# cuulee/reporter

Measured on AMD Instinct MI355X. Metric: GPS probes matched/sec (whole node), higher is better.
Workload: dtype f64; 1 GPU; c2; graph=metro, nodes=1048576, directed_edges=3527937, osmlr_segments=1361487, traces_per_gpu=10000, streams=1, device_batches=1, output_segments=1688548

## Files before the change

### reporter_amd/csrc/otr_device.h

```cpp
#pragma once
#include <hip/hip_runtime.h>
#include <stdint.h>

#include "../../include/otr_graph_format.h"

#define OTR_KMAX 64
#define OTR_MODES 3
#define OTR_WAVE 64
#define OTR_COUNTERS 24

namespace otr {

constexpr double kMetersPerDeg = 20037581.187 / 180.0;

struct MatchParams {
  double sigma_z;
  double beta;
  double max_route_distance_factor;
  double breakage_distance;
  double interpolation_distance;
  double search_radius;
  double max_search_radius;
  double gps_accuracy;
  double max_route_time_factor;
  double turn_penalty_factor;
  double speed_kph;
  double queue_kph;
  double inv2s2;
  double inv_beta;
  int32_t kmax;
  int32_t pad;
};

struct ModeParams {
  MatchParams m[OTR_MODES];
  double delta;
};

constexpr double kMaxBreakage = 30000.0;
constexpr int64_t kTbMax = 131070;
constexpr uint32_t kTcCap = 2097151;

__host__ __device__ inline int32_t time_bound_ds(const MatchParams& p, int64_t dt) {
  if (!(p.max_route_time_factor > 0.0) || dt <= 0) return -1;
  const double b = floor(p.max_route_time_factor * (double)dt * 10.0);
  return b <= (double)kTbMax ? (int32_t)b : -1;
}

__host__ __device__ inline int turn_from_back(int back, int hb_begin) {
  int td = hb_begin - back;
  td += td < 0 ? 360 : 0;
  return td <= 180 ? td : 360 - td;
}
__host__ __device__ inline int heading_back(int ha_end) { return ha_end >= 180 ? ha_end - 180 : ha_end + 180; }
__host__ __device__ inline int turn_degree(int ha_end, int hb_begin) {
  return turn_from_back(heading_back(ha_end), hb_begin);
}

struct DevGraph {
  const uint32_t* node_row;
  const uint32_t* rev_row;
  const uint32_t* rev_edge;
  const uint32_t* edge_src;
  const uint32_t* edge_dst;
  const float* edge_len;
  const uint32_t* edge_attr;
  const uint32_t* edge_shape;
  const uint32_t* edge_seg;
  const uint32_t* edge_way;
  const int2* shape_ll;
  const unsigned long long* seg_id;
  const uint32_t* seg_len;
  const uint32_t* cell_row;
  const uint32_t* cell_edge;
  const uint4* cell_rec;
  const uint4* edge_pack;
  const uint4* eprep;
  const uint4* adj;
  const uint32_t* node_minin;
  const uint32_t* len_mm;
  const int2* node_ll;
  const uint32_t* adj_t;
  const uint32_t* edge_t;
  uint32_t adj_t_stride, edge_t_stride;
  const short2* edge_head;
  const uint2* adj_e;
  const uint4* erec;
  const uint32_t* erec_t;
  size_t erec_stride;
  uint32_t n_nodes, n_edges, n_segments, grid_rows, grid_cols;
  double grid_min_lat, grid_min_lon, grid_cell_deg;
  __device__ const uint32_t* et(int mode) const { return edge_t + (size_t)mode * edge_t_stride; }
};

__host__ __device__ inline double cos_deg(double deg) {
  double x = deg * (3.14159265358979323846 / 180.0);
  double x2 = x * x;
  double r = -1.0 / 1124000727777607680000.0;
  r = r * x2 + 1.0 / 2432902008176640000.0;
  r = r * x2 - 1.0 / 6402373705728000.0;
  r = r * x2 + 1.0 / 20922789888000.0;
  r = r * x2 - 1.0 / 87178291200.0;
  r = r * x2 + 1.0 / 479001600.0;
  r = r * x2 - 1.0 / 3628800.0;
  r = r * x2 + 1.0 / 40320.0;
  r = r * x2 - 1.0 / 720.0;
  r = r * x2 + 1.0 / 24.0;
  r = r * x2 - 1.0 / 2.0;
  r = r * x2 + 1.0;
  return r;
}

__host__ __device__ inline double gc_dist(double lat1, double lon1, double lat2, double lon2) {
  double x = (lon1 - lon2) * kMetersPerDeg * cos_deg(0.5 * (lat1 + lat2));
  double y = (lat1 - lat2) * kMetersPerDeg;
  return sqrt(x * x + y * y);
}

__host__ __device__ inline double e6(int32_t v) { return (double)v * 1e-6; }

__host__ __device__ inline double route_bound(const MatchParams& p, double g) {
  double gf = g > p.interpolation_distance ? g : p.interpolation_distance;
  double b = p.max_route_distance_factor * gf;
  return b > p.breakage_distance ? p.breakage_distance : b;
}

__device__ inline uint32_t hmix(uint32_t x) {
  x ^= x >> 16;
  x *= 0x7feb352dU;
  x ^= x >> 15;
  x *= 0x846ca68bU;
  x ^= x >> 16;
  return x;
}

__device__ inline int lane_id() { return (int)__lane_id(); }

__device__ inline int64_t xcd_remap(int64_t b, int64_t per) { return (b & 7) * per + (b >> 3); }

struct XcdQueue {
  int64_t lo, hi;
  unsigned long long* ctr;
  __device__ XcdQueue(unsigned long long* q, int64_t n) {
    const int parts = gridDim.x >= 8 ? 8 : 1;
    const int x = parts == 8 ? (int)(blockIdx.x & 7) : 0;
    const int64_t per = (n + parts - 1) / parts;
    lo = (int64_t)x * per;
    hi = lo + per < n ? lo + per : n;
    ctr = q + 16 * x;
  }
  __device__ unsigned long long claim() {
    unsigned long long v = 0;
    if (threadIdx.x == 0) v = atomicAdd(ctr, 1ull);
    return v;
  }
  __device__ int64_t take(unsigned long long v) const {
    const uint32_t l = (uint32_t)__builtin_amdgcn_readfirstlane((int)(uint32_t)v);
    const uint32_t h = (uint32_t)__builtin_amdgcn_readfirstlane((int)(uint32_t)(v >> 32));
    return lo + (int64_t)(((unsigned long long)h << 32) | l);
  }
  __device__ int64_t next() { return take(claim()); }
};

__device__ inline uint4 ld16(const uint4* p) {
  uint4 r = *p;
  asm volatile("" : "+v"(r.x), "+v"(r.y), "+v"(r.z), "+v"(r.w));
  return r;
}

constexpr int kShards = 64;
constexpr int kCShards = 256;
__device__ inline int cshard() { return (int)(blockIdx.x & (kCShards - 1)); }
constexpr uint32_t kAdjDstMask = 0x0FFFFFFFu;
constexpr uint32_t kAdjMore = 0x80000000u;

// ... 6 lines not shown
```

### reporter_amd/csrc/otr_engine.hip

```cpp
#include <hipcub/hipcub.hpp>

#include <cerrno>
#include <cstdio>
#include <cstring>
#include <fcntl.h>
#include <sys/mman.h>
#include <sys/stat.h>
#include <unistd.h>

#include "otr_engine.h"
#include "otr_kernels.h"
#include "otr_edge.h"
#include "otr_edge1.h"
#include "otr_ingest.h"
#include "otr_launch.h"
#include "otr_points.h"
#include "otr_traversals.h"

namespace otr {
static_assert(kTraceWaves == 4, "grid_trace_rows (otr_launch.h) assumes 4 traces per block");

#define HIPCHK(x)                                                                        \
  do {                                                                                   \
    hipError_t e_ = (x);                                                                 \
    if (e_ != hipSuccess) {                                                              \
      if (err) *err = std::string("HIP error: ") + hipGetErrorString(e_) + " at " #x;    \
      return OTR_DEVICE_ERROR;                                                           \
    }                                                                                    \
  } while (0)

void finalize_params(MatchParams* p) {
  p->inv2s2 = 1.0 / (p->sigma_z * p->sigma_z * 2.0);
  p->inv_beta = 1.0 / p->beta;
  if (p->kmax > OTR_KMAX) p->kmax = OTR_KMAX;
  if (p->kmax < 1) p->kmax = 1;
}

const char* check_params(const MatchParams& p) {
  if (!(p.breakage_distance >= 0.0 && p.breakage_distance <= kMaxBreakage))
    return "breakage_distance must be within [0, 30000] m";
  if (!(p.max_route_distance_factor >= 0.0) || !(p.max_route_distance_factor < 1e6))
    return "max_route_distance_factor must be >= 0";
  if (!(p.max_route_time_factor >= 0.0) || !(p.max_route_time_factor < 1e6)) return "max_route_time_factor must be >= 0";
  if (!(p.turn_penalty_factor >= 0.0) || !(p.turn_penalty_factor <= 1e6)) return "turn_penalty_factor must be within [0, 1e6]";
  if (!(p.sigma_z > 0.0)) return "sigma_z must be > 0";
  if (!(p.beta > 0.0)) return "beta must be > 0";
  if (!(p.search_radius >= 0.0) || !(p.max_search_radius >= 0.0)) return "search_radius must be >= 0";
  if (!(p.interpolation_distance >= 0.0)) return "interpolation_distance must be >= 0";
  if (!(p.speed_kph >= 0.0) || !(p.queue_kph >= 0.0)) return "speed_kph and queue_kph must be >= 0";
  return nullptr;
}

ModeParams default_mode_params() {
  ModeParams mp{};
  for (int m = 0; m < OTR_MODES; ++m) {
    MatchParams& p = mp.m[m];
    p.sigma_z = 4.07;
    p.beta = 3.0;
    p.max_route_distance_factor = 5.0;
    p.max_route_time_factor = 2.0;
    p.breakage_distance = 2000.0;
    p.interpolation_distance = 10.0;
    p.search_radius = 50.0;
    p.max_search_radius = 100.0;
    p.gps_accuracy = 5.0;
    p.kmax = 32;
    p.queue_kph = 10.0;
  }
  mp.m[0].turn_penalty_factor = 200.0;
  mp.m[1].turn_penalty_factor = 140.0;
  mp.m[1].speed_kph = 18.0;
  mp.m[1].queue_kph = 5.0;
  mp.m[2].turn_penalty_factor = 100.0;
  mp.m[2].speed_kph = 5.1;
  mp.m[2].queue_kph = 2.0;
  for (int m = 0; m < OTR_MODES; ++m) finalize_params(&mp.m[m]);
  mp.delta = 60.0;
  return mp;
}

static uint32_t edge_time_ds(uint32_t attr, uint32_t len_mm, double speed_cap) {
  double kph = (double)OTR_ATTR_SPEED(attr);
  if (!(kph > 0.0)) kph = 30.0;
  if (speed_cap > 0.0 && speed_cap < kph) kph = speed_cap;
  const double v = (double)len_mm * 0.036 / kph;
  return v < 2.0e9 ? (uint32_t)llround(v) : 2000000000u;
}

static int seg_heading(const int32_t* a, const int32_t* b) {
  const double la1 = (double)a[0] * 1e-6, lo1 = (double)a[1] * 1e-6;
  const double la2 = (double)b[0] * 1e-6, lo2 = (double)b[1] * 1e-6;
  const double m = 20037581.187 / 180.0;
  const double x = (lo2 - lo1) * m * cos_deg(0.5 * (la1 + la2));
// ... 34 lines not shown
};
struct Staged {
  std::vector<void*> allocs;
  bool adopted = false;
  ~Staged() {
    if (!adopted)
      for (void* q : allocs) (void)hipFree(q);
  }
};
}

int engine_configure(const Config& cfg, std::string* err) {
  for (int m = 0; m < OTR_MODES; ++m)
    if (const char* bad = check_params(cfg.mp.m[m])) {
      if (err) *err = std::string("config: ") + bad;
      return OTR_BAD_REQUEST;
    }
  int fd = open(cfg.graph_path.c_str(), O_RDONLY);
  if (fd < 0) {
    if (err) *err = "cannot open graph file " + cfg.graph_path + ": " + strerror(errno);
    return OTR_BAD_REQUEST;
  }
  struct stat st;
  fstat(fd, &st);
  Mapped mf;
  mf.n = (size_t)st.st_size;
  mf.p = mf.n >= sizeof(otr_graph_header) ? mmap(nullptr, mf.n, PROT_READ, MAP_PRIVATE, fd, 0) : MAP_FAILED;
  close(fd);
  if (mf.p == MAP_FAILED) {
    if (err) *err = "cannot map graph file " + cfg.graph_path;
    return OTR_BAD_REQUEST;
  }
  const char* base = (const char*)mf.p;
  otr_graph_header h;
  memcpy(&h, base, sizeof(h));
  if (memcmp(h.magic, OTR_GRAPH_MAGIC, 8) != 0 || h.version != OTR_GRAPH_VERSION ||
      h.array_offset[OTR_A_END] > (uint64_t)st.st_size) {
    if (err) *err = "not an OTR graph file: " + cfg.graph_path;
    return OTR_BAD_REQUEST;
  }
  if (h.n_nodes >= (1u << 28)) {
    if (err) *err = "graph has more than 2^28 nodes";
    return OTR_BAD_REQUEST;
  }
  if (h.n_edges >= (1u << 28)) {
    if (err) *err = "graph has more than 2^28 directed edges";
    return OTR_BAD_REQUEST;
  }
  const uint32_t* dst = (const uint32_t*)(base + h.array_offset[OTR_A_EDGE_DST]);
  const float* lenf = (const float*)(base + h.array_offset[OTR_A_EDGE_LEN]);
  const uint32_t* attr = (const uint32_t*)(base + h.array_offset[OTR_A_EDGE_ATTR]);
  const uint32_t* row = (const uint32_t*)(base + h.array_offset[OTR_A_NODE_ROW]);
  const int32_t* nll = (const int32_t*)(base + h.array_offset[OTR_A_NODE_LL]);
  const uint32_t* eshape = (const uint32_t*)(base + h.array_offset[OTR_A_EDGE_SHAPE]);
  const int32_t* sll = (const int32_t*)(base + h.array_offset[OTR_A_SHAPE_LL]);
  std::vector<uint32_t> len(h.n_edges + 1, 0u);
  for (uint32_t e = 0; e < h.n_edges; ++e) {
    const double mm = (double)lenf[e] * 1000.0;
    if (!(mm >= 0.0 && mm < 2.0e9)) {
      if (err) *err = "graph edge length outside [0, 2000 km)";
      return OTR_BAD_REQUEST;
    }
    len[e] = (uint32_t)std::max(1LL, (long long)llround(mm));
  }
  for (uint32_t u = 0; u < h.n_nodes; ++u)
    if (row[u + 1] < row[u] || row[u + 1] > h.n_edges) {
      if (err) *err = "graph CSR rows are not monotone";
      return OTR_BAD_REQUEST;
    }
  for (uint32_t e = 0; e < h.n_edges; ++e)
    if (dst[e] >= h.n_nodes || eshape[e + 1] < eshape[e] + 2 || eshape[e + 1] > h.n_shape) {
      if (err) *err = "graph edge " + std::to_string(e) + " has a bad end node or shape range";
      return OTR_BAD_REQUEST;
    }
  std::vector<uint32_t> minin(h.n_nodes + 1, 0xFFFFFFFFu);
  for (uint32_t e = 0; e < h.n_edges; ++e) minin[dst[e]] = std::min(minin[dst[e]], len[e]);
  std::vector<uint4> pack(h.n_edges + 1);
  for (uint32_t e = 0; e < h.n_edges; ++e) pack[e] = make_uint4(dst[e], len[e], attr[e], minin[dst[e]]);
  std::vector<uint4> eprep(h.n_edges + 1, make_uint4(0u, 0u, 0u, 0u));
  {
    const uint32_t* srcv = (const uint32_t*)(base + h.array_offset[OTR_A_EDGE_SRC]);
    for (uint32_t e = 0; e < h.n_edges; ++e) eprep[e] = make_uint4(len[e], srcv[e], minin[srcv[e]], dst[e]);
  }
  std::vector<uint4> adj(4ull * h.n_nodes + 4, make_uint4(kAdjDstMask, 0u, 0u, 0u));
  for (uint32_t u = 0; u < h.n_nodes; ++u) {
    const uint32_t deg = row[u + 1] - row[u];
    for (uint32_t k = 0; k < deg && k < 4; ++k) {
      const uint32_t e = row[u] + k;
      adj[4ull * u + k] = make_uint4(dst[e] | ((attr[e] & OTR_ATTR_ACCESS_MASK) << 28), len[e], minin[dst[e]], 0u);
    }
    if (deg > 4) adj[4ull * u + 3].x |= kAdjMore;
  }
  std::vector<uint32_t> et[OTR_MODES], at[OTR_MODES];
  for (int m = 0; m < OTR_MODES; ++m) {
    et[m].assign(h.n_edges + 1, 0u);
    for (uint32_t e = 0; e < h.n_edges; ++e) et[m][e] = edge_time_ds(attr[e], len[e], cfg.mp.m[m].speed_kph);
    at[m].assign(4ull * h.n_nodes + 4, 0u);
    for (uint32_t u = 0; u < h.n_nodes; ++u)
      for (uint32_t k = 0; k < 4 && row[u] + k < row[u + 1]; ++k) at[m][4ull * u + k] = et[m][row[u] + k];
  }
  std::vector<short2> head(h.n_edges + 1, make_short2(0, 0));
  for (uint32_t e = 0; e < h.n_edges; ++e) {
    const uint32_t k0 = eshape[e], k1 = eshape[e + 1];
    int hb = -1, he = -1;
    for (uint32_t k = k0; k + 1 < k1 && hb < 0; ++k) hb = seg_heading(sll + 2ull * k, sll + 2ull * k + 2);
    for (uint32_t k = k1 - 1; k > k0 && he < 0; --k) he = seg_heading(sll + 2ull * k - 2, sll + 2ull * k);
    head[e] = make_short2((short)(hb < 0 ? 0 : hb), (short)(he < 0 ? 0 : he));
  }
  std::vector<uint2> adje(4ull * h.n_nodes + 4, make_uint2(0u, 0u));
  for (uint32_t u = 0; u < h.n_nodes; ++u)
    for (uint32_t k = 0; k < 4 && row[u] + k < row[u + 1]; ++k) {
      const uint32_t e = row[u] + k;
      adje[4ull * u + k] = make_uint2(e, (uint32_t)(uint16_t)head[e].x | ((uint32_t)(uint16_t)head[e].y << 16));
    }
  const size_t es = 4ull * h.n_edges + 4;
  std::vector<uint4> erec(es, make_uint4(kAdjDstMask, 0u, 0u, 0u));
  std::vector<uint32_t> erec_t(es * OTR_MODES, 0u);
  for (uint32_t b = 0; b < h.n_edges; ++b) {
    const uint32_t v = dst[b], deg = row[v + 1] - row[v];
    for (uint32_t k = 0; k < 4; ++k) {
      const uint32_t hend = (uint32_t)(uint16_t)head[b].y << 8;
      if (k >= deg) {
        erec[4ull * b + k] = make_uint4(kAdjDstMask, 0u, hend, v);
        continue;
      }
      const uint32_t e = row[v] + k;
      const uint32_t x = e | ((attr[e] & OTR_ATTR_ACCESS_MASK) << 28) | ((k == 3 && deg > 4) ? kAdjMore : 0u);
      erec[4ull * b + k] =
          make_uint4(x, len[e], (uint32_t)turn_degree((int)head[b].y, (int)head[e].x) | hend, v);
      for (int m = 0; m < OTR_MODES; ++m) erec_t[es * m + 4ull * b + k] = std::min(et[m][e], 0x1FFFFu);
    }
  }
  const uint32_t* cedge = (const uint32_t*)(base + h.array_offset[OTR_A_CELL_EDGE]);
  std::vector<uint4> crec(3 * ((size_t)h.n_cell_entries + 1), make_uint4(0u, 0u, 0u, 0u));
  for (uint64_t q = 0; q < h.n_cell_entries; ++q) {
    const uint32_t e = cedge[q];
    if (e >= h.n_edges) {
      if (err) *err = "graph cell index names a missing edge";
      return OTR_BAD_REQUEST;
    }
    const uint32_t k0 = eshape[e], k1 = eshape[e + 1];
    crec[3 * q] = make_uint4(e, k0, k1, attr[e]);
    uint32_t pt[8] = {0u, 0u, 0u, 0u, 0u, 0u, 0u, 0u};
    for (uint32_t i = 0; i < 4 && k0 + i < k1; ++i) {
      pt[2 * i] = (uint32_t)sll[2ull * (k0 + i)];
      pt[2 * i + 1] = (uint32_t)sll[2ull * (k0 + i) + 1];
    }
    crec[3 * q + 1] = make_uint4(pt[0], pt[1], pt[2], pt[3]);
    crec[3 * q + 2] = make_uint4(pt[4], pt[5], pt[6], pt[7]);
  }
  HIPCHK(hipSetDevice(cfg.device));
  Staged sg;
  bool alloc_ok = true;
  auto upv = [&](const void* src, size_t bytes) -> void* {
    void* d = nullptr;
    if (hipMalloc(&d, bytes ? bytes : 16) != hipSuccess) {
      alloc_ok = false;
      return nullptr;
    }
    sg.allocs.push_back(d);
    if (bytes && hipMemcpy(d, src, bytes, hipMemcpyHostToDevice) != hipSuccess) alloc_ok = false;
    return d;
  };
  auto up = [&](int a, size_t bytes) -> void* { return upv(base + h.array_offset[a], bytes); };
  DevGraph g{};
  g.node_row = (const uint32_t*)up(OTR_A_NODE_ROW, 4ull * (h.n_nodes + 1));
  g.rev_row = (const uint32_t*)up(OTR_A_REV_ROW, 4ull * (h.n_nodes + 1));
  g.node_ll = (const int2*)up(OTR_A_NODE_LL, 8ull * h.n_nodes);
  g.rev_edge = (const uint32_t*)up(OTR_A_REV_EDGE, 4ull * h.n_edges);
  g.edge_src = (const uint32_t*)up(OTR_A_EDGE_SRC, 4ull * h.n_edges);
  g.edge_dst = (const uint32_t*)up(OTR_A_EDGE_DST, 4ull * h.n_edges);
  g.edge_len = (const float*)up(OTR_A_EDGE_LEN, 4ull * h.n_edges);
  g.edge_attr = (const uint32_t*)up(OTR_A_EDGE_ATTR, 4ull * h.n_edges);
  g.edge_shape = (const uint32_t*)up(OTR_A_EDGE_SHAPE, 4ull * (h.n_edges + 1));
  g.edge_seg = (const uint32_t*)up(OTR_A_EDGE_SEG, 4ull * h.n_edges);
  g.edge_way = (const uint32_t*)up(OTR_A_EDGE_WAY, 4ull * h.n_edges);
  g.shape_ll = (const int2*)up(OTR_A_SHAPE_LL, 8ull * h.n_shape);
  g.seg_id = (const unsigned long long*)up(OTR_A_SEG_ID, 8ull * h.n_segments);
  g.seg_len = (const uint32_t*)up(OTR_A_SEG_LEN, 4ull * h.n_segments);
  g.cell_row = (const uint32_t*)up(OTR_A_CELL_ROW, 4ull * (h.n_cells + 1));
  g.cell_edge = (const uint32_t*)up(OTR_A_CELL_EDGE, 4ull * h.n_cell_entries);
  g.len_mm = (const uint32_t*)upv(len.data(), 4ull * len.size());
  g.edge_pack = (const uint4*)upv(pack.data(), sizeof(uint4) * pack.size());
// ... 2681 lines not shown
```

### reporter_amd/csrc/otr_kernels.h

```cpp
#pragma once
#include <cstddef>
#include <type_traits>

#include "otr_device.h"
#include "otr_mincode.h"
#include "otr_pred.h"
#include "otr_report.h"
#include "otr_tilerow.h"

#ifndef OTR_CAP1
#define OTR_CAP1 160
#endif
#ifndef OTR_LOAD1
#define OTR_LOAD1 7
#endif
#ifndef OTR_E1CAP
#define OTR_E1CAP 360
#endif
#ifndef OTR_E1LOAD
#define OTR_E1LOAD 14
#endif

namespace otr {

// ... 693 lines not shown
  const typename LabelT<LM>::T old = atomicMin(&L.lab[sl], nb);
  if (LabelT<LM>::label(nb) < LabelT<LM>::label(old)) {
    knext = nd < knext ? nd : knext;
    if constexpr (OLD) {
      const uint32_t ok = atomicOr(&L.key[sl], kInq);
      if (!(ok & kInq)) return sl;
    } else {
      if (old == LabelT<LM>::kInf) return sl;
    }
  }
  return -1;
}

template <int CAP, bool OLD = false>
__device__ inline int relax_sink(SearchLds<CAP, 0>& L, uint32_t* sink, const Pack& K, uint32_t dw, uint32_t len_mm,
                                 uint32_t time_ds, uint32_t minin, uint32_t pu, uint32_t pd, uint32_t pt,
                                 uint32_t mode_bit, uint32_t& relaxed, uint32_t& knext, bool& isnew, uint32_t& lanew) {
  const bool mode_ok = (((dw >> 28) & 7u) & mode_bit) != 0u;
  relaxed += mode_ok ? 1u : 0u;
  const uint32_t nd = K.d(pu) + len_mm;
  const uint32_t tt = K.t(pu) + time_ds;
  const uint32_t nw = (nd << K.sh) | tt;
  const uint32_t node = dw & kAdjDstMask;
  bool go = mode_ok && nd <= pd && tt <= pt;
  uint32_t* mine = sink + lane_id();
  const uint32_t h0 = hslot<CAP>(node);
  const uint32_t k0 = atomicCAS(go ? &L.key[h0] : mine, kEmpty, node);
  isnew = go && k0 == kEmpty;
  int sl = (go && (k0 == kEmpty || (k0 & kNodeMask) == node)) ? (int)h0 : -1;
  const bool coll = go && sl < 0;
  if (__ballot(coll) != 0ull) {
    if (coll) {
      uint32_t hh = h0;
      for (int probe = 1; probe < CAP; ++probe) {
        hh = hh + 1 == (uint32_t)CAP ? 0u : hh + 1;
        const uint32_t k = atomicCAS(&L.key[hh], kEmpty, node);
        if (k == kEmpty) {
          isnew = true;
          sl = (int)hh;
          break;
        }
        if ((k & kNodeMask) == node) {
          sl = (int)hh;
          break;
        }
      }
      if (sl < 0) {
        L.overflow = 1;
        lanew |= kProbeOut;
      }
    }
  }
  go = go && sl >= 0;
  using MiT = typename SearchLds<CAP, 0>::MiT;
  *((go && isnew) ? &L.mi[sl] : reinterpret_cast<MiT*>(mine)) = SearchLds<CAP, 0>::code(minin);
  const uint32_t old = atomicMin(go ? &L.lab[sl] : mine, nw);
  const bool imp = go && nw < old;
  knext = (imp && nd < knext) ? nd : knext;
  if constexpr (OLD) {
    const uint32_t was = atomicOr(imp ? &L.key[sl] : mine, kInq);
    return (imp && !(was & kInq)) ? sl : -1;
  } else {
    return (imp && old == kNoLabel) ? sl : -1;
  }
}

struct NDump {
  const unsigned long long* in;
  unsigned long long* base;
  unsigned long long* ctr;
  uint32_t words, slots;
#ifdef OTR_FORCE_RETRY
  int stop_rounds;
#endif
};
__host__ __device__ constexpr uint32_t nd_words(int cap) { return 2u + (uint32_t)cap + ((uint32_t)cap + 1u) / 2u; }
#ifndef OTR_ND_IN_MIN
#define OTR_ND_IN_MIN 2048
#endif
#ifndef OTR_ND_OUT_MIN
#define OTR_ND_OUT_MIN 1024
#endif

template <int CAP, int LM, int G = 1, bool RIN = false, bool ROUT = false>
__device__ bool search_run(SearchLds<CAP, LM>* Ls, const DevGraph& g, const Pack& K, uint32_t mode_bit, bool active,
                           uint32_t start, uint32_t pd, uint32_t pt, uint32_t tnode, uint32_t tpart, uint32_t gapT,
                           int n_tgt, unsigned long long* settled, unsigned long long* relaxed,
                           unsigned long long* rounds, unsigned long long* stamps = nullptr, uint32_t* sink = nullptr,
                           const NDump* nd = nullptr, int* dslot = nullptr) {
  using Gr = Grp<G>;
  constexpr bool OLD = old_rounds(G);
  static_assert(!(OLD && (RIN || ROUT)), "the dump and resume code assumes keys without the pending bit");
  constexpr int kMaxKeys = (CAP <= 128 || CAP >= 256) ? (CAP * 7) / 8 : (CAP * OTR_LOAD1) / 8;
  const int gl = Gr::gl();
  using W = typename LabelT<LM>::W;
  SearchLds<CAP, LM>& L = Ls[Gr::g()];
  using Idx = typename SearchLds<CAP, LM>::Idx;
  constexpr int WCAP = SearchLds<CAP, LM>::WCAP;
  const bool timed = K.sh != 0u;
  const uint32_t* adjt = g.adj_t + (size_t)__builtin_ctz(mode_bit) * g.adj_t_stride;
  uint32_t kmin = 0;
  int npend = active ? 1 : 0;
  const bool resume = RIN && LM == 0 && active && nd->in != nullptr;
  const int nres = resume ? (int)nd->in[0] : 0;
  const int nrx = RIN ? Gr::umax(nres) : 0;
  if (RIN && nrx > 0) {
    const unsigned long long* D = nd->in;
    const uint32_t* M = (const uint32_t*)(D + 2 + nres);
    int np = 0;
    for (int base = 0; base < nrx; base += Gr::GL) {
      const int k = base + gl;
      bool pend = false;
      int sl = 0;
      if (k < nres) {
        const unsigned long long e = D[2 + k];
        const uint32_t key = (uint32_t)(e >> 32), node = key & kNodeMask;
        uint32_t h = hslot<CAP>(node);
        for (int probe = 0; probe < CAP; ++probe) {
          if (atomicCAS(&L.key[h], kEmpty, node) == kEmpty) break;
          h = h + 1 == (uint32_t)CAP ? 0u : h + 1;
        }
        sl = (int)h;
        L.key[sl] = key & ~kInq;
        L.lab[sl] = (typename LabelT<LM>::T)(uint32_t)e;
        L.mi[sl] = SearchLds<CAP, LM>::code(M[k]);
        pend = (key & kInq) != 0u;
      }
      const unsigned long long mp = __ballot(pend);
      if (pend && np + Gr::prefix(mp) < SearchLds<CAP, LM>::PCAP) L.pend[np + Gr::prefix(mp)] = (Idx)sl;
      np += Gr::count(mp);
    }
    if (resume && np > SearchLds<CAP, LM>::PCAP) {
      if (gl == 0) L.overflow = 1;
      np = SearchLds<CAP, LM>::PCAP;
    }
    if (resume) {
      npend = np;
      kmin = (uint32_t)D[1];
      if (gl == 0) L.n_keys = nres;
    }
  }
  if (!resume && active && gl == 0) {
    bool isnew;
    const int sl = lds_insert(L, start, &isnew);
    L.mi[sl] = 0;
    L.lab[sl] = LabelT<LM>::make(0u, kEmpty);
    if (OLD) L.key[sl] |= kInq;
    L.pend[0] = (Idx)sl;
  }
  __syncthreads();
  int tslot = -1;
  if (active && gl < n_tgt && tnode != kEmpty) {
    bool isnew;
    tslot = lds_insert(L, tnode, &isnew);
    if (tslot >= 0 && isnew) L.mi[tslot] = SearchLds<CAP, LM>::code(gapT);
  }
  __syncthreads();
  uint32_t my_settled = 0, my_relaxed = 0, my_rounds = 0;
  unsigned long long cyc[4] = {0, 0, 0, 0};
  bool done = !active, grew = false;
#ifdef OTR_FORCE_RETRY
  int force_round = 0;
#endif
  int nkeys = 0;
  constexpr bool AHEAD = !OLD && LM != 1;
  static_assert(!AHEAD || Gr::GL <= SearchLds<CAP, LM>::PCAP, "the first pending chunk lies inside the list");
  const int ts = tslot < 0 ? 0 : tslot;
  int p0 = 0;
  bool ovf = false;
  uint32_t tkey = 0u;
  typename LabelT<LM>::T tlab = LabelT<LM>::kInf;
  if constexpr (AHEAD) {
    nkeys = L.n_keys;
    ovf = L.overflow != 0;
    tkey = L.key[ts];
    tlab = L.lab[ts];
    p0 = (int)L.pend[gl];
  }
  for (;;) {
    OTR_STAMP(t0);
    const int np = done ? 0 : npend;
    OTR_STAMP(t1);
    bool res;
    if constexpr (AHEAD)
      res = done | (gl >= n_tgt) |
            target_test<LM, OLD>(tkey, LabelT<LM>::label(tlab), K, tslot, tpart, gapT, pd, kmin, np == 0);
    else
      res = done | (gl >= n_tgt) | target_resolved<CAP, LM, OLD>(L, K, tslot, tpart, gapT, pd, kmin, np == 0);
    done = done || Gr::mine(__ballot(!res)) == 0ull || np == 0;
    OTR_STAMP(t2);
    cyc[0] += t1 - t0;
    cyc[1] += t2 - t1;
    if (Gr::all(done)) break;
    if (!done && gl == 0) ++my_rounds;
    uint32_t knext = 0xFFFFFFFFu;
    int kept = 0, nw = 0;
    const int npx = OLD ? Gr::umax(np) : 0;
    for (int base = 0; OLD ? base < npx : __ballot(base + gl < np) != 0ull; base += Gr::GL) {
      const int k = base + gl;
      const bool in = k < np;
      int sl;
      if constexpr (AHEAD) {
        int pk = p0;
        if (base != 0) pk = (int)L.pend[k];
        sl = in ? pk : 0;
      } else {
        sl = in ? (int)L.pend[k] : 0;
      }
      const W lb = LabelT<LM>::label(L.lab[sl]);
      const uint32_t key = L.key[sl];
      const uint32_t d = K.d(lb);
      bool take, keep;
      if constexpr (OLD) {
        take = in && (uint64_t)d < (uint64_t)kmin + SearchLds<CAP, LM>::gap(L.mi[sl]);
        take = take && nw + Gr::prefix(__ballot(take)) < WCAP;
        keep = in && !take;
      } else {
        const uint32_t gp = SearchLds<CAP, LM>::gap(L.mi[sl]);
        if constexpr (LM != 2) take = in & in_final32(d, kmin, gp);
        else take = in & ((uint64_t)d < (uint64_t)kmin + gp);
        take = take & (nw + Gr::prefix(__ballot(take)) < WCAP);
        keep = in & !take;
      }
      const unsigned long long mt = __ballot(take), mk = __ballot(keep);
      __syncthreads();
      if (take) {
        L.work[nw + Gr::prefix(mt)] = WorkE<W>{key & kNodeMask, lb};
        L.key[sl] = (key & kNodeMask) | kRel;
      }
      if (keep) L.pend[kept + Gr::prefix(mk)] = (Idx)sl;
      knext = (keep && d < knext) ? d : knext;
      nw += Gr::count(mt);
      kept += Gr::count(mk);
      __syncthreads();
    }
    npend = kept;
    OTR_STAMP(t3);
    cyc[2] += t3 - t2;
    uint32_t tail = 0u;
    uint32_t unread = 0u;
    uint32_t& lanew = AHEAD ? tail : unread;
    const int nwx = OLD ? Gr::umax(4 * nw) : 0;
    for (int base = 0; OLD ? base < nwx : __ballot(base + gl < 4 * nw) != 0ull; base += Gr::GL) {
      const int k = base + gl;
      int psl = -1;
      bool isnew = false;
      if (k < 4 * nw) {
        const WorkE<W> wk = L.work[k >> 2];
        const uint32_t wnode = wk.node;
        const int slot = k & 3;
        if (slot == 0) ++my_settled;
        const uint32_t tq = adjt[4 * (size_t)wnode + slot];
        const uint4 r = ld16(g.adj + 4 * (size_t)wnode + slot);
        const uint32_t tt = timed ? tq : 0u;
        if constexpr (LM == 0) {
#ifdef OTR_NO_SINK
          psl = relax_one<CAP, LM, false, OLD>(L, K, r.x & ~kAdjMore, r.y, tt, r.z, wk.lab, 0u, pd, pt, mode_bit,
                                               my_relaxed, knext, isnew, lanew);
#else
          psl = relax_sink<CAP, OLD>(L, sink, K, r.x & ~kAdjMore, r.y, tt, r.z, wk.lab, pd, pt, mode_bit, my_relaxed,
                                     knext, isnew, lanew);
#endif
        } else {
          const uint32_t e0 = LM == 1 ? g.node_row[wnode] : 0u;
          psl = relax_one<CAP, LM, false, OLD>(L, K, r.x & ~kAdjMore, r.y, tt, r.z, wk.lab, e0 + slot, pd, pt,
                                               mode_bit, my_relaxed, knext, isnew, lanew);
        }
        tail |= slot == 3 ? (r.x & kAdjMore) : 0u;
      }
      nkeys += Gr::count(__ballot(isnew));
      const unsigned long long mp = __ballot(psl >= 0);
#ifndef OTR_NO_SINK
      if constexpr (LM == 0 && G == 1) {
        const int p = npend + Gr::prefix(mp);
        constexpr int PC = SearchLds<CAP, LM>::PCAP;
        *(psl >= 0 ? &L.pend[p < PC ? p : PC - 1] : reinterpret_cast<Idx*>(sink + lane_id())) = (Idx)psl;
      } else
#endif
      if (psl >= 0) {
        const int p = npend + Gr::prefix(mp);
        L.pend[p < SearchLds<CAP, LM>::PCAP ? p : SearchLds<CAP, LM>::PCAP - 1] = (Idx)psl;
      }
      npend += Gr::count(mp);
    }
    if (SearchLds<CAP, LM>::PCAP < CAP && npend > SearchLds<CAP, LM>::PCAP) {
      if (gl == 0) L.overflow = 1;
      npend = SearchLds<CAP, LM>::PCAP;
      ovf = true;
    }
    if (__ballot(AHEAD ? (tail & kAdjMore) != 0u : tail != 0u) != 0ull) {
      if (gl == 0) L.n_pend = npend;
      if (AHEAD && gl == 0) L.n_keys = nkeys;
      __syncthreads();
      for (int base = 0; OLD ? base < nwx : __ballot(base + gl < 4 * nw) != 0ull; base += Gr::GL) {
        const int k = base + gl;
        if (k < 4 * nw && (k & 3) == 3) {
          const WorkE<W> wk = L.work[k >> 2];
          const uint32_t wnode = wk.node;
          if (g.adj[4 * (size_t)wnode + 3].x & kAdjMore)
            for (uint32_t e = g.node_row[wnode] + 4; e < g.node_row[wnode + 1]; ++e) {
              const uint4 pk = ld16(g.edge_pack + e);
              const uint32_t tt = timed ? g.et(__builtin_ctz(mode_bit))[e] : 0u;
              bool isnew;
              const int psl = relax_one<CAP, LM, true, OLD>(L, K, pk.x | ((pk.z & 7u) << 28), pk.y, tt, pk.w, wk.lab, e,
                                                            pd, pt, mode_bit, my_relaxed, knext, isnew, lanew);
              if (psl >= 0) {
                const int p = atomicAdd(&L.n_pend, 1);
                if (p < SearchLds<CAP, LM>::PCAP) L.pend[p] = (Idx)psl;
                else L.overflow = 1;
              }
            }
        }
      }
      __syncthreads();
      npend = L.n_pend;
      if (npend > SearchLds<CAP, LM>::PCAP) npend = SearchLds<CAP, LM>::PCAP;
      if constexpr (AHEAD) {
        nkeys = L.n_keys;
        ovf = ovf || L.overflow != 0;
      }
    }
    __syncthreads();
    if constexpr (AHEAD) {
      tkey = L.key[ts];
      tlab = L.lab[ts];
      p0 = (int)L.pend[gl];
      ovf = ovf || Gr::mine(__ballot((tail & kProbeOut) != 0u)) != 0ull;
    }
    OTR_STAMP(t4);
    cyc[3] += t4 - t3;
    const uint32_t km = Gr::min_u32(knext);
    if (!done) kmin = km;
    const int keys = AHEAD ? nkeys : L.n_keys + nkeys;
    const bool over = AHEAD ? ovf : L.overflow != 0;
    if (!done && (over || keys > kMaxKeys)) {
      grew = !over && keys > kMaxKeys;
      done = true;
    }
#ifdef OTR_FORCE_RETRY
    ++force_round;
    if (ROUT && !done && nd->base != nullptr && nd->stop_rounds > 0 && force_round >= nd->stop_rounds &&
        !over) {
      grew = true;
      done = true;
    }
#endif
    if constexpr (!AHEAD) __syncthreads();
    if (done && active && gl == 0 && (keys > kMaxKeys || grew)) L.overflow = 1;
  }
  if constexpr (AHEAD) {
    if (gl == 0) L.n_keys = nkeys;
  } else {
    if (gl == 0) L.n_keys += nkeys;
  }
  if (ROUT) *dslot = -1;
  if (ROUT && LM == 0 && __ballot(grew && active && nd->base != nullptr) != 0ull) {
    int v = 0;
    if (grew && active && nd->base != nullptr && gl == 0) v = (int)atomicAdd(nd->ctr, 1ull);
    v = __shfl(v, 0, Gr::GL);
    const bool dump = grew && active && nd->base != nullptr && (uint32_t)v < nd->slots;
    unsigned long long* D = dump ? nd->base + (size_t)v * nd->words : nullptr;
    int n = 0;
    for (int base = 0; base < CAP; base += Gr::GL) {
      const int k = base + gl;
      const uint32_t key = (dump && k < CAP) ? L.key[k] : kEmpty;
      const bool has = key != kEmpty;
      const unsigned long long m = __ballot(has);
      if (has) {
        const uint32_t lb = (uint32_t)L.lab[k];
        const uint32_t kq = (lb != kNoLabel && !(key & kRel)) ? key | kInq : key;
        D[2 + n + Gr::prefix(m)] = (unsigned long long)lb | ((unsigned long long)kq << 32);
      }
      n += Gr::count(m);
    }
    uint32_t* M = dump ? (uint32_t*)(D + 2 + n) : nullptr;
    int q = 0;
    for (int base = 0; base < CAP; base += Gr::GL) {
      const int k = base + gl;
      const bool has = dump && k < CAP && L.key[k] != kEmpty;
      const unsigned long long m = __ballot(has);
      if (has) M[q + Gr::prefix(m)] = SearchLds<CAP, LM>::gap(L.mi[k]);
      q += Gr::count(m);
    }
    if (dump && gl == 0) {
      D[0] = (unsigned long long)(uint32_t)n;
      D[1] = kmin;
    }
    *dslot = dump ? v : -1;
  }
#ifdef OTR_STAMPS
  if (stamps && threadIdx.x == 0)
    for (int q = 0; q < 4; ++q) atomicAdd(&stamps[q * kCShards + cshard()], cyc[q]);
#endif
  if (settled) *settled += my_settled;
  if (relaxed) *relaxed += my_relaxed;
  if (rounds) *rounds += my_rounds;
  __syncthreads();
  return !L.overflow;
}

struct PrepArgs {
  int64_t n_states;
  const int64_t* prev;
  const double* bound;
  const int32_t* cand_count;
  const uint32_t* cand_edge;
  const double* cand_p;
  const int32_t* state_trace;
  const uint8_t* mode;
  uint4* cprep;
  uint2* cprep_t;
  uint2* clen;
  int32_t* nroot;
  uint32_t turn_modes;
};

template <int G>
__global__ __launch_bounds__(256) void k_prep(DevGraph g, PrepArgs a) {
  constexpr int GL = OTR_WAVE / G;
  const int64_t s = ((int64_t)blockIdx.x * (blockDim.x / OTR_WAVE) + threadIdx.x / OTR_WAVE) * G +
                    (threadIdx.x % OTR_WAVE) / GL;
  const int lane = threadIdx.x % GL;
  if (s >= a.n_states) return;
  const int K = a.cand_count[s];
  if (K <= 0) return;
  const int md = a.mode[a.state_trace[s]] < OTR_MODES ? a.mode[a.state_trace[s]] : 0;
  const bool turn = (a.turn_modes >> md) & 1u;
  uint32_t root = 0xFFFFFFFFu, t0 = 0u;
  if (lane < K) {
    const uint32_t e = a.cand_edge[s * OTR_KMAX + lane];
    const double p = a.cand_p[s * OTR_KMAX + lane];
    const uint4 ep = g.eprep[e];
    const uint32_t et = g.et(md)[e];
// ... 240 lines not shown
      trec[Gr::g()][1] = r1;
      trec[Gr::g()][2] = r2;
    }
    const int64_t s = r0.x;
    const unsigned long long mask = ((unsigned long long)r1.w << 32) | r1.z;
    const int64_t sp = r0.y;
    Kb = (int)(r1.y & 0xFFu);
    K.sh = (r1.y >> 11) & 31u;
    const bool general = (r1.y >> 16) & 1u;
    fits = Kb <= Gr::GL && (WIDE || !general) && !((r1.y >> 17) & 1u);
    const bool pre = G >= 2 && !LIST && have && ((r1.y >> 18) & 1u);
    if (pre) {
      start_tier = (int)((r1.y >> 19) & 7u);
      fits = false;
    }
    mode_bit = 1u << ((r1.y >> 8) & 3u);
    bmm = r0.w;
    root = r0.z;
    d0min = r1.x;
    const int32_t bt = (int32_t)r2.y;
    bool needed = false;
    uint4 cq = make_uint4(0u, 0u, 0u, 0u);
    if (have && !pre && lane < Kb) {
      ej = a.cand_edge[s * OTR_KMAX + lane];
      pj = a.cand_p[s * OTR_KMAX + lane];
      cq = a.cprep[s * OTR_KMAX + lane];
      tpart = cq.x;
    }
    const int nsrc = have && !pre ? __popcll(mask) : 0;
    iq = lane < nsrc ? nth_set_bit(mask, lane) : 0;
    if (lane < nsrc) {
      e_q = a.cand_edge[sp * OTR_KMAX + iq];
      p_q = a.cand_p[sp * OTR_KMAX + iq];
      if (bt >= 0) t_q = a.cprep_t[sp * OTR_KMAX + iq].y;
    }
    for (int q = 0; q < nsrc; ++q) {
      uint32_t ei;
      double pi;
      if (q < Gr::GL) {
        ei = (uint32_t)__shfl((int)e_q, q, Gr::GL);
        pi = __shfl(p_q, q, Gr::GL);
      } else {
        const int i = nth_set_bit(mask, q);
        ei = a.cand_edge[sp * OTR_KMAX + i];
        pi = a.cand_p[sp * OTR_KMAX + i];
      }
      if (lane < Kb && !(ej == ei && pj >= pi)) needed = true;
    }
    const uint32_t t0 = (uint32_t)__shfl((int)t_q, 0, Gr::GL);
    bool feasible_root = d0min <= bmm;
    pd = feasible_root ? bmm - d0min : 0u;
    if (bt >= 0) {
      feasible_root = feasible_root && t0 <= (uint32_t)bt;
      pt = t0 <= (uint32_t)bt ? (uint32_t)bt - t0 : 0u;
    }
    forced = have && ((r1.y >> 10) & 1u);
    const unsigned long long need_mask = __ballot(needed);
    search = have && fits && !forced && feasible_root && Gr::mine(need_mask) != 0ull;
    if (needed) {
      tnode = cq.y;
      gapT = cq.z ? cq.z : 1u;
    }
  }
  unsigned long long settled = 0, relaxed = 0, rounds = 0;
  OTR_STAMP(ts_set);
  NDump nd{};
  int dslot = -1;
  constexpr bool kIn = LIST && !WIDE && CAP >= OTR_ND_IN_MIN, kOut = LIST && !WIDE && CAP >= OTR_ND_OUT_MIN;
  constexpr bool kDumps = kIn || kOut;
  if (kIn) {
    const int32_t rs = (a.dump_in != nullptr && search) ? a.task_dump[task] : -1;
    nd.in = rs >= 0 ? a.dump_in + (size_t)rs * a.dump_in_words : nullptr;
  }
  if (kOut) {
    nd.base = a.dump_out;
    nd.ctr = a.dump_ctr;
    nd.words = a.dump_out_words;
    nd.slots = a.dump_out_slots;
#ifdef OTR_FORCE_RETRY
    nd.stop_rounds = (a.force_edge >> 7) & 1 ? 2 + Gr::g() : 0;
#endif
  }
  search_init<CAP, LM, G>(Ls);
  bool ok = search_run<CAP, LM, G, kIn, kOut>(Ls, gr, K, mode_bit, search, root, pd, pt, tnode, tpart, gapT, Kb, &settled,
                                   &relaxed, &rounds, counters ? counters + 16 * kCShards : nullptr, sink,
                                   kDumps ? &nd : nullptr, kDumps ? &dslot : nullptr) &&
            fits;
#ifdef OTR_FORCE_RETRY
  if (G >= 2 && !LIST) ok = false;
#endif
  OTR_STAMP(ts_srch);
  SearchLds<CAP, LM>& L = Ls[Gr::g()];
  int64_t lab = -1;
  if (ok && search && tnode != kEmpty && !forced) {
    const int sl = lds_find(L, tnode);
    if (sl >= 0 && LabelT<LM>::label(L.lab[sl]) != LabelT<LM>::kNone) lab = (int64_t)LabelT<LM>::label(L.lab[sl]);
  }
  asm volatile("" ::: "memory");
  uint32_t ntr = 0;
  if (have && forced && Kb > Gr::GL) {
    const uint4 r1 = trec[Gr::g()][1], r2 = trec[Gr::g()][2];
    const unsigned long long mask = ((unsigned long long)r1.w << 32) | r1.z;
    uint32_t* trow = a.trans + (int64_t)(((uint64_t)r2.w << 32) | r2.z);
    for (int q = 0; q < __popcll(mask); ++q) {
      const int i = nth_set_bit(mask, q);
      for (int j = lane; j < Kb; j += Gr::GL) trow[(int64_t)i * Kb + j] = kNoRoute;
    }
  } else if (have && (ok || forced)) {
    const uint4 r0 = trec[Gr::g()][0], r1 = trec[Gr::g()][1], r2 = trec[Gr::g()][2];
    const int64_t s = r0.x;
    const unsigned long long mask = ((unsigned long long)r1.w << 32) | r1.z;
    if (search) ntr = (uint32_t)Kb * (uint32_t)__popcll(mask);
    const int64_t sp = r0.y;
    const int32_t bt = (int32_t)r2.y;
    uint32_t* trow = a.trans + (int64_t)(((uint64_t)r2.w << 32) | r2.z);
    const int nsrc = __popcll(mask);
    uint32_t w_q = 0;
    uint2 l_q = make_uint2(0u, 0u);
    if (!kKeep) {
      if (!LIST) {
        e_q = t_q = ej = 0u;
        p_q = pj = 0.0;
      }
      iq = lane < nsrc ? nth_set_bit(mask, lane) : 0;
    }
    if (lane < nsrc) {
      if (!kKeep) {
        e_q = a.cand_edge[sp * OTR_KMAX + iq];
        p_q = a.cand_p[sp * OTR_KMAX + iq];
        if (bt >= 0) t_q = a.cprep_t[sp * OTR_KMAX + iq].y;
      }
      w_q = a.cprep[sp * OTR_KMAX + iq].w;
      l_q = a.clen[sp * OTR_KMAX + iq];
    }
    uint32_t tpt = 0;
    if (lane < Kb) {
      if (!kKeep) {
        ej = a.cand_edge[s * OTR_KMAX + lane];
        pj = a.cand_p[s * OTR_KMAX + lane];
      }
      tpt = bt >= 0 ? a.cprep_t[s * OTR_KMAX + lane].x : 0u;
    }
    for (int q = 0; q < nsrc; ++q) {
      int i;
      uint32_t ei, wi, ti, li, lti;
      double pi;
      if (q < Gr::GL) {
        i = __shfl(iq, q, Gr::GL);
        ei = (uint32_t)__shfl((int)e_q, q, Gr::GL);
        pi = __shfl(p_q, q, Gr::GL);
        wi = (uint32_t)__shfl((int)w_q, q, Gr::GL);
        ti = (uint32_t)__shfl((int)t_q, q, Gr::GL);
        li = (uint32_t)__shfl((int)l_q.x, q, Gr::GL);
        lti = (uint32_t)__shfl((int)l_q.y, q, Gr::GL);
      } else {
        i = nth_set_bit(mask, q);
        ei = a.cand_edge[sp * OTR_KMAX + i];
        pi = a.cand_p[sp * OTR_KMAX + i];
        wi = a.cprep[sp * OTR_KMAX + i].w;
        ti = bt >= 0 ? a.cprep_t[sp * OTR_KMAX + i].y : 0u;
        const uint2 l = a.clen[sp * OTR_KMAX + i];
        li = l.x;
        lti = l.y;
      }
      if (lane < Kb) {
        int64_t r = -1, rt = 0;
        if (forced) {
          r = -1;
        } else if (ej == ei && pj >= pi) {
          r = part_mm(pj - pi, li);
          if (bt >= 0) rt = part_mm(pj - pi, lti);
        } else if (lab >= 0) {
          r = (int64_t)wi + K.d((uint64_t)lab) + tpart;
          if (bt >= 0) rt = (int64_t)ti + K.t((uint64_t)lab) + tpt;
        }
        const bool valid = r >= 0 && r <= (int64_t)bmm && (bt < 0 || rt <= (int64_t)bt);
        trow[(int64_t)i * Kb + lane] = valid ? (uint32_t)r : kNoRoute;
      }
    }
// ... 1161 lines not shown
```

Baseline: 37.00 million probes/s.

## Fold per-mode edge times into adjacency records and reuse tracked target label

Builds one adjacency block per travel mode with the edge time stored in the record's fourth word. The search inner loop then needs one 16-byte load per relaxed edge instead of that load plus a separate adj_t load. It also passes back the target label already tracked during the look-ahead search, so the LDS hash lookup after the search can be skipped. The cost is three times the adjacency memory footprint, and the new label path relies on tslot/tlab being correct.

```diff
diff --git a/reporter_amd/csrc/otr_adj.h b/reporter_amd/csrc/otr_adj.h
--- /dev/null
+++ b/reporter_amd/csrc/otr_adj.h
@@ -0,0 +1,25 @@
+#pragma once
+#include <cstddef>
+#include <cstdint>
+
+#include "otr_device.h"
+
+namespace otr {
+
+inline size_t adj_block_size(uint32_t n_nodes) { return 4ull * n_nodes + 4; }
+
+inline void fill_adj_block(uint4* out, uint32_t n_nodes, const uint32_t* row, const uint32_t* dst,
+                           const uint32_t* attr, const uint32_t* len_mm, const uint32_t* minin, const uint32_t* et) {
+  const size_t n = adj_block_size(n_nodes);
+  for (size_t i = 0; i < n; ++i) out[i] = make_uint4(kAdjDstMask, 0u, 0u, 0u);
+  for (uint32_t u = 0; u < n_nodes; ++u) {
+    const uint32_t deg = row[u + 1] - row[u];
+    for (uint32_t k = 0; k < deg && k < 4; ++k) {
+      const uint32_t e = row[u] + k;
+      out[4ull * u + k] = adj_record(dst[e], attr[e] & OTR_ATTR_ACCESS_MASK, len_mm[e], minin[dst[e]], et[e]);
+    }
+    if (deg > 4) out[4ull * u + 3].x |= kAdjMore;
+  }
+}
+
+}
diff --git a/reporter_amd/csrc/otr_device.h b/reporter_amd/csrc/otr_device.h
--- a/reporter_amd/csrc/otr_device.h
+++ b/reporter_amd/csrc/otr_device.h
@@ -57,6 +57,11 @@
   return turn_from_back(heading_back(ha_end), hb_begin);
 }
 
+__host__ __device__ inline uint4 adj_record(uint32_t dst, uint32_t access, uint32_t len_mm, uint32_t minin_dst,
+                                            uint32_t time_ds) {
+  return make_uint4(dst | (access << 28), len_mm, minin_dst, time_ds);
+}
+
 struct DevGraph {
   const uint32_t* node_row;
   const uint32_t* rev_row;
@@ -91,6 +96,7 @@
   uint32_t n_nodes, n_edges, n_segments, grid_rows, grid_cols;
   double grid_min_lat, grid_min_lon, grid_cell_deg;
   __device__ const uint32_t* et(int mode) const { return edge_t + (size_t)mode * edge_t_stride; }
+  __device__ const uint4* adj_m(int mode) const { return adj + (size_t)mode * adj_t_stride; }
 };
 
 __host__ __device__ inline double cos_deg(double deg) {
diff --git a/reporter_amd/csrc/otr_engine.hip b/reporter_amd/csrc/otr_engine.hip
--- a/reporter_amd/csrc/otr_engine.hip
+++ b/reporter_amd/csrc/otr_engine.hip
@@ -9,6 +9,7 @@
 #include <unistd.h>
 
 #include "otr_engine.h"
+#include "otr_adj.h"
 #include "otr_kernels.h"
 #include "otr_edge.h"
 #include "otr_edge1.h"
@@ -209,15 +210,6 @@
     const uint32_t* srcv = (const uint32_t*)(base + h.array_offset[OTR_A_EDGE_SRC]);
     for (uint32_t e = 0; e < h.n_edges; ++e) eprep[e] = make_uint4(len[e], srcv[e], minin[srcv[e]], dst[e]);
   }
-  std::vector<uint4> adj(4ull * h.n_nodes + 4, make_uint4(kAdjDstMask, 0u, 0u, 0u));
-  for (uint32_t u = 0; u < h.n_nodes; ++u) {
-    const uint32_t deg = row[u + 1] - row[u];
-    for (uint32_t k = 0; k < deg && k < 4; ++k) {
-      const uint32_t e = row[u] + k;
-      adj[4ull * u + k] = make_uint4(dst[e] | ((attr[e] & OTR_ATTR_ACCESS_MASK) << 28), len[e], minin[dst[e]], 0u);
-    }
-    if (deg > 4) adj[4ull * u + 3].x |= kAdjMore;
-  }
   std::vector<uint32_t> et[OTR_MODES], at[OTR_MODES];
   for (int m = 0; m < OTR_MODES; ++m) {
     et[m].assign(h.n_edges + 1, 0u);
@@ -226,6 +218,10 @@
     for (uint32_t u = 0; u < h.n_nodes; ++u)
       for (uint32_t k = 0; k < 4 && row[u] + k < row[u + 1]; ++k) at[m][4ull * u + k] = et[m][row[u] + k];
   }
+  const size_t as = adj_block_size(h.n_nodes);
+  std::vector<uint4> adj(as * OTR_MODES);
+  for (int m = 0; m < OTR_MODES; ++m)
+    fill_adj_block(adj.data() + as * m, h.n_nodes, row, dst, attr, len.data(), minin.data(), et[m].data());
   std::vector<short2> head(h.n_edges + 1, make_short2(0, 0));
   for (uint32_t e = 0; e < h.n_edges; ++e) {
     const uint32_t k0 = eshape[e], k1 = eshape[e + 1];
diff --git a/reporter_amd/csrc/otr_kernels.h b/reporter_amd/csrc/otr_kernels.h
--- a/reporter_amd/csrc/otr_kernels.h
+++ b/reporter_amd/csrc/otr_kernels.h
@@ -799,12 +799,14 @@
 #define OTR_ND_OUT_MIN 1024
 #endif
 
+__host__ __device__ constexpr bool search_ahead(int G, int LM) { return !old_rounds(G) && LM != 1; }
 template <int CAP, int LM, int G = 1, bool RIN = false, bool ROUT = false>
 __device__ bool search_run(SearchLds<CAP, LM>* Ls, const DevGraph& g, const Pack& K, uint32_t mode_bit, bool active,
                            uint32_t start, uint32_t pd, uint32_t pt, uint32_t tnode, uint32_t tpart, uint32_t gapT,
                            int n_tgt, unsigned long long* settled, unsigned long long* relaxed,
                            unsigned long long* rounds, unsigned long long* stamps = nullptr, uint32_t* sink = nullptr,
-                           const NDump* nd = nullptr, int* dslot = nullptr) {
+                           const NDump* nd = nullptr, int* dslot = nullptr,
+                           typename LabelT<LM>::W* tlabel = nullptr) {
   using Gr = Grp<G>;
   constexpr bool OLD = old_rounds(G);
   static_assert(!(OLD && (RIN || ROUT)), "the dump and resume code assumes keys without the pending bit");
@@ -815,7 +817,12 @@
   using Idx = typename SearchLds<CAP, LM>::Idx;
   constexpr int WCAP = SearchLds<CAP, LM>::WCAP;
   const bool timed = K.sh != 0u;
+#ifdef OTR_ADJT_LOAD
+  const uint4* adjm = g.adj;
   const uint32_t* adjt = g.adj_t + (size_t)__builtin_ctz(mode_bit) * g.adj_t_stride;
+#else
+  const uint4* adjm = g.adj_m(__builtin_ctz(mode_bit));
+#endif
   uint32_t kmin = 0;
   int npend = active ? 1 : 0;
   const bool resume = RIN && LM == 0 && active && nd->in != nullptr;
@@ -880,7 +887,7 @@
   int force_round = 0;
 #endif
   int nkeys = 0;
-  constexpr bool AHEAD = !OLD && LM != 1;
+  constexpr bool AHEAD = search_ahead(G, LM);
   static_assert(!AHEAD || Gr::GL <= SearchLds<CAP, LM>::PCAP, "the first pending chunk lies inside the list");
   const int ts = tslot < 0 ? 0 : tslot;
   int p0 = 0;
@@ -967,8 +974,13 @@
         const uint32_t wnode = wk.node;
         const int slot = k & 3;
         if (slot == 0) ++my_settled;
+#ifdef OTR_ADJT_LOAD
         const uint32_t tq = adjt[4 * (size_t)wnode + slot];
-        const uint4 r = ld16(g.adj + 4 * (size_t)wnode + slot);
+        const uint4 r = ld16(adjm + 4 * (size_t)wnode + slot);
+#else
+        const uint4 r = ld16(adjm + 4 * (size_t)wnode + slot);
+        const uint32_t tq = r.w;
+#endif
         const uint32_t tt = timed ? tq : 0u;
         if constexpr (LM == 0) {
 #ifdef OTR_NO_SINK
@@ -1066,6 +1078,7 @@
     if (done && active && gl == 0 && (keys > kMaxKeys || grew)) L.overflow = 1;
   }
   if constexpr (AHEAD) {
+    if (tlabel) *tlabel = tslot >= 0 ? LabelT<LM>::label(tlab) : LabelT<LM>::kNone;
     if (gl == 0) L.n_keys = nkeys;
   } else {
     if (gl == 0) L.n_keys += nkeys;
@@ -1472,9 +1485,15 @@
 #endif
   }
   search_init<CAP, LM, G>(Ls);
+#ifdef OTR_FIND_LABEL
+  constexpr bool kLabel = false;
+#else
+  constexpr bool kLabel = search_ahead(G, LM);
+#endif
+  typename LabelT<LM>::W tlw = LabelT<LM>::kNone;
   bool ok = search_run<CAP, LM, G, kIn, kOut>(Ls, gr, K, mode_bit, search, root, pd, pt, tnode, tpart, gapT, Kb, &settled,
                                    &relaxed, &rounds, counters ? counters + 16 * kCShards : nullptr, sink,
-                                   kDumps ? &nd : nullptr, kDumps ? &dslot : nullptr) &&
+                                   kDumps ? &nd : nullptr, kDumps ? &dslot : nullptr, kLabel ? &tlw : nullptr) &&
             fits;
 #ifdef OTR_FORCE_RETRY
   if (G >= 2 && !LIST) ok = false;
@@ -1483,8 +1502,12 @@
   SearchLds<CAP, LM>& L = Ls[Gr::g()];
   int64_t lab = -1;
   if (ok && search && tnode != kEmpty && !forced) {
-    const int sl = lds_find(L, tnode);
-    if (sl >= 0 && LabelT<LM>::label(L.lab[sl]) != LabelT<LM>::kNone) lab = (int64_t)LabelT<LM>::label(L.lab[sl]);
+    if constexpr (kLabel) {
+      if (tlw != LabelT<LM>::kNone) lab = (int64_t)tlw;
+    } else {
+      const int sl = lds_find(L, tnode);
+      if (sl >= 0 && LabelT<LM>::label(L.lab[sl]) != LabelT<LM>::kNone) lab = (int64_t)LabelT<LM>::label(L.lab[sl]);
+    }
   }
   asm volatile("" ::: "memory");
   uint32_t ntr = 0;
```

Result: no change. 37.33 million probes/s, median of 6 (+0.9%).
